# daveredrum/D3Net

Hardware: AMD Instinct MI355X
Metric: scenes/sec fwd+bwd (PointGroup+speaker) (higher is better)
Workload: dtype bf16

## Files before the change

### d3net_amd/_lib.py

```python
import ctypes as C
import os

_HERE = os.path.dirname(os.path.abspath(__file__))
SO_PATH = os.path.join(_HERE, "lib", "libd3hip.so")

ERRORS = {-1: "D3_ERR_WORKSPACE", -2: "D3_ERR_RANGE (coordinate/batch outside key range)",
          -3: "D3_ERR_ARG", -4: "D3_ERR_OVERFLOW"}


class D3Error(RuntimeError):
    pass


_lib = None
vp, i32, i64, f32, sz = C.c_void_p, C.c_int, C.c_longlong, C.c_float, C.c_size_t
f64 = C.c_double
pi = C.POINTER(C.c_int)

SIGNATURES = {
    "d3_version": (i32, []),
    "d3_arch": (C.c_char_p, []),
    "d3_sec_mean": (i32, [vp, vp, vp, i32, i32, vp]),
    "d3_sec_min": (i32, [vp, vp, vp, i32, i32, vp]),
    "d3_sec_max": (i32, [vp, vp, vp, i32, i32, vp]),
# ... 145 lines not shown
    "d3_multiview_fuse_ws_bytes": (sz, [i32, i32, i32]),
    "d3_multiview_fuse": (i32, [vp, i32, vp, vp, vp, i32, C.POINTER(f64), i32, i32, vp, i32, i32, vp, vp, vp, sz, vp]),
    "d3_enet_layers": (i32, [vp, i32]),
    "d3_enet_param_count": (i64, []),
    "d3_enet_preprocess": (i32, [vp, i32, i32, i32, vp, vp, i32, i32, vp, vp]),
    "d3_enet_ws_bytes": (sz, [i32, i32, i32]),
    "d3_enet_forward": (i32, [vp, i32, i32, i32, vp, i64, vp, i32, i32, vp, vp, sz, vp]),
    "d3_scan_limits": (i32, [pi, pi, pi, pi, pi]),
    "d3_scan_mesh_ws_bytes": (sz, [i32, i32]),
    "d3_scan_mesh": (i32, [vp, i32, vp, i32, C.POINTER(f64), vp, vp, vp, vp, sz, vp]),
    "d3_scan_labels_ws_bytes": (sz, [i32, i32, i32, i32, i32]),
    "d3_scan_labels": (i32, [vp, vp, i32, i32, vp, vp, i32, vp, vp, i32, i32, vp, vp, vp, vp, vp, vp, vp, vp, vp, sz, vp]),
    "d3_cider_ws_bytes": (sz, [i32, i32, i32]),
    "d3_cider_scores": (i32, [vp, i32, vp, vp, vp, vp, vp, i32, i32, vp, i32, vp, i32, i32, f64, i32, vp, vp, vp, sz, vp]),
    "d3_graph_edges": (i32, [vp, vp, i32, i32, i32, vp, vp, vp, vp, vp, vp, vp, vp, vp, vp, vp]),
    "d3_edgeconv_ws_bytes": (sz, [i32, i32, i32]),
    "d3_edgeconv_bwd_ws_bytes": (sz, [i32, i32, i32]),
    "d3_edgeconv_fwd": (i32, [vp, vp, vp, vp, vp, vp, vp, vp, vp, i32, i32, i32, i32, i32, vp, vp, vp, sz, vp]),
    "d3_edgeconv_bwd": (i32, [vp, vp, vp, vp, vp, vp, vp, vp, i32, i32, i32, i32, i32, vp, vp, vp, vp, vp, vp, vp, vp, vp, sz, vp]),
    "d3_query_locals_dist": (i32, [vp, vp, vp, i32, i32, i32, f32, i32, vp]),
    "d3_prof_enable": (i32, [i32]),
    "d3_net_set_chunks": (i32, [vp, vp, i32]),
    "d3_net_chunk_wait": (i32, [vp, i32, vp]),
    "d3_layernorm_fwd": (i32, [vp, vp, vp, vp, vp, vp, vp, i32, i32, f32, vp]),
    "d3_layernorm_ws_bytes": (sz, [i32, i32]),
    "d3_layernorm_bwd": (i32, [vp, vp, vp, vp, vp, vp, vp, vp, vp, i32, i32, vp, sz, vp]),
    "d3_tuning_set": (i32, [C.c_char_p, i32]),
    "d3_tuning_get": (i32, [C.c_char_p, vp]),
    "d3_tuning_count": (i32, []),
    "d3_tuning_name": (C.c_char_p, [i32]),
    "d3_prof_collect": (i32, [i32, C.POINTER(C.c_longlong), C.POINTER(C.c_double), C.POINTER(C.c_double),
                              C.POINTER(C.c_double)]),
    "d3_prof_dump": (i32, [i32, C.POINTER(C.c_double), i32, C.POINTER(i32)]),
    "d3_bn_ws_bytes": (sz, [i32]),
    "d3_bn_stats": (i32, [vp, i32, i32, vp, vp, vp, vp, f32, vp, sz, vp]),
    "d3_bn_relu_fwd": (i32, [vp, vp, vp, vp, vp, vp, i32, i32, f32, i32, vp]),
    "d3_bn_relu_fwd_bf16": (i32, [vp, vp, vp, vp, vp, vp, i32, i32, f32, i32, vp]),
    "d3_bn_relu_bwd": (i32, [vp, vp, vp, vp, vp, vp, vp, vp, vp, i32, i32, f32, i32, vp, sz, vp]),
}


class GemmSeg(C.Structure):
    _fields_ = [("A", vp), ("ia", vp), ("lda", i64), ("a_kmajor", i32), ("B", vp), ("ldb", i64), ("b_kmajor", i32), ("K", i32)]


class GemmProb(C.Structure):
# ... 63 lines not shown
```

### d3net_amd/csrc/unet.hip

```cpp
#include "conv.h"
#include <vector>
#include <map>
#include <string.h>
#include <stdlib.h>

__device__ __forceinline__ unsigned int un_pack2bf(float lo, float hi) {
    unsigned int a = __float_as_uint(lo), b = __float_as_uint(hi);
    a += 0x7FFFu + ((a >> 16) & 1u); b += 0x7FFFu + ((b >> 16) & 1u);
    return (a >> 16) | (b & 0xFFFF0000u);
}

__device__ __forceinline__ float un_ld1(const float *p, long long idx, int bf) {
    return bf ? __uint_as_float((unsigned int)((const unsigned short *)p)[idx] << 16) : p[idx];
}
__device__ __forceinline__ float4 un_ldx4(const float *x, long long idx, int xbf) {
    if (xbf) { const uint2 v = *(const uint2 *)((const unsigned short *)x + idx); return make_float4(__uint_as_float(v.x), __uint_as_float(v.y), 0.f, 0.f); }
    return *(const float4 *)(x + idx);
}
__device__ __forceinline__ void un_cvx4(const float4 r, int xbf, float *o) {
    if (xbf) {
        const unsigned int a = __float_as_uint(r.x), b = __float_as_uint(r.y);
        o[0] = __uint_as_float(a << 16); o[1] = __uint_as_float(a & 0xFFFF0000u); o[2] = __uint_as_float(b << 16); o[3] = __uint_as_float(b & 0xFFFF0000u);
    } else { o[0] = r.x; o[1] = r.y; o[2] = r.z; o[3] = r.w; }
}
// ... 543 lines not shown
}

enum { OP_CONV = 1, OP_BNACT = 2, OP_PADCAST = 3, OP_STATS = 4 };
enum { MAP_K1 = 0, MAP_K3 = 1, MAP_DOWN = 2, MAP_UP = 3 };

struct TensorD { int level, C, ld, coff, dtype, buf; };
struct BufD { int level, width, dtype; size_t off, goff; int need_grad; };
struct SrcRef { int op, c0, cn; };
struct OpD {
    int type, in, out, res, w, gamma, beta, rmean, rvar, map, mlevel, K, CinW, stats, relu;
    float eps, momentum;
    int Cin, Cout;
    size_t wp_fwd, wp_bwd, part_off, state_off;
    int nparts, partw;
    std::vector<SrcRef> srcs;
    int in_grad_mode;
    int res_mode;
    int needs_dgrad_pack;
    int bn_of_in;
    int fused_by;
    size_t bpart_off; int bparts;
    size_t part2_off, bpart2_off;
    int wg_hazard;
    size_t wpart_off, wpart_bytes; int wsplits;
    int use_shadow;
    int write_shadow;
};
#define RED_RING 32
struct Net {
    std::vector<TensorD> T;
    std::vector<BufD> B;
    std::vector<OpD> ops;
    int nlevels = 0, nparams = 0, input_needs_grad = 0, out_tensor = -1;
    std::vector<int> rows;
    std::vector<int> galias;
    std::vector<int> gbf;
    std::vector<int> gabf;
    std::vector<int> gshadow;
    std::vector<size_t> gshadow_off;
    size_t arena_bytes = 0, grad_bytes = 0, ws_bytes = 0, bnscr_off = 0, wgws_off = 0, bnscr_bytes = 0, wgws_bytes = 0;
    bool planned = false;
    bool f32 = false;
    size_t cnt_off0 = 0, cnt_bytes = 0, bcnt_off0 = 0, bcnt_bytes = 0;
    std::vector<PackJob> jobs;
    PackJob *jobs_dev = nullptr;
    size_t jobs_cap = 0;
    long long pack_total = 0;
    hipStream_t side = nullptr;
    hipStream_t side2 = nullptr;
    std::vector<hipEvent_t> ev;
    size_t ev_used = 0;
    int xp_op = -1;
    int xp_tensor = -1;
    const void *xp_ext = nullptr;
    std::vector<const void *> k3_16;
    std::vector<const void *> k3_q;
    std::vector<int> chunk_op;
    std::vector<hipEvent_t> chunk_ev_side, chunk_ev_main;
    RedJob *red_host = nullptr, *red_dev = nullptr;
    size_t red_cap = 0; int red_flip = 0;
    hipEvent_t next_event() {
        if (ev_used == ev.size()) { hipEvent_t e; if (hipEventCreateWithFlags(&e, hipEventDisableTiming) != hipSuccess) return nullptr; ev.push_back(e); }
        return ev[ev_used++];
    }
};

static int esize(int dtype) { return dtype == 1 ? 2 : 4; }

extern "C" void *d3_net_create(const int64_t *prog, int nops, const int64_t *tensors, int ntensors, const int64_t *bufs,
                               int nbufs, int nlevels, int nparams, int input_needs_grad, int out_tensor) {
    Net *n = new Net();
    n->nlevels = nlevels; n->nparams = nparams; n->input_needs_grad = input_needs_grad; n->out_tensor = out_tensor;
    for (int i = 0; i < ntensors; i++) {
        const int64_t *t = tensors + (size_t)i * 6;
        n->T.push_back(TensorD{(int)t[0], (int)t[1], (int)t[2], (int)t[3], (int)t[4], (int)t[5]});
    }
    for (int i = 0; i < nbufs; i++) {
        const int64_t *b = bufs + (size_t)i * 3;
        n->B.push_back(BufD{(int)b[0], (int)b[1], (int)b[2], 0, 0, 1});
    }
    n->f32 = true;
    for (auto &b : n->B) if (b.dtype == 1) n->f32 = false;
    for (int i = 0; i < nops; i++) {
        const int64_t *p = prog + (size_t)i * 16;
        OpD o;
        o.type = (int)p[0]; o.in = (int)p[1]; o.out = (int)p[2]; o.res = (int)p[3];
        o.w = o.gamma = o.beta = o.rmean = o.rvar = -1; o.map = 0; o.mlevel = 0; o.K = 1; o.CinW = 0; o.stats = 0; o.relu = 0;
        o.eps = 0.f; o.momentum = 0.f; o.Cin = o.Cout = 0; o.wp_fwd = o.wp_bwd = o.part_off = o.state_off = 0;
        o.nparts = 0; o.partw = 0; o.in_grad_mode = 0; o.res_mode = 0; o.needs_dgrad_pack = 0;
        o.bn_of_in = -1; o.fused_by = -1; o.bpart_off = 0; o.bparts = 0; o.part2_off = 0; o.bpart2_off = 0; o.wg_hazard = 0; o.wpart_off = 0; o.wpart_bytes = 0; o.wsplits = 1; o.use_shadow = 0; o.write_shadow = 0;
        if (o.type == OP_CONV) {
            o.w = (int)p[4]; o.map = (int)p[5]; o.mlevel = (int)p[6]; o.K = (int)p[7]; o.CinW = (int)p[8]; o.stats = (int)p[9];
            o.Cin = n->T[o.in].C; o.Cout = n->T[o.out].C;
        } else if (o.type == OP_BNACT) {
            o.gamma = (int)p[4]; o.beta = (int)p[5]; o.rmean = (int)p[6]; o.rvar = (int)p[7]; o.relu = (int)p[8];
            int32_t eb = (int32_t)p[9], mb = (int32_t)p[10];
            memcpy(&o.eps, &eb, 4); memcpy(&o.momentum, &mb, 4);
        } else if (o.type == OP_STATS) {
            o.stats = 1;
        }
        if (o.type == OP_PADCAST && n->xp_op < 0 && n->T[(size_t)o.in].buf < 0) { n->xp_op = (int)n->ops.size(); n->xp_tensor = o.out; }
        n->ops.push_back(o);
    }
    for (auto &o : n->ops) {
        if (o.type != OP_BNACT) continue;
        const TensorD &ti = n->T[o.in];
        for (size_t j = 0; j < n->ops.size(); j++) {
            const OpD &p = n->ops[j];
            if (!p.stats) continue;
            const TensorD &tp = n->T[p.type == OP_STATS ? p.in : p.out];
            if (tp.buf != ti.buf) continue;
            if (tp.coff >= ti.coff && tp.coff + tp.C <= ti.coff + ti.C) o.srcs.push_back(SrcRef{(int)j, tp.coff - ti.coff, tp.C});
        }
// ... 132 lines not shown
        };
        struct LastBn { int op, coff, C; };
        std::map<int, LastBn> last_bn;
        for (int i = (int)n->ops.size() - 1; on && i >= 0; i--) {
            OpD &o = n->ops[i];
            int coff, C;
            if (o.type == OP_CONV) {
                const int ro = root_of(o.out, coff, C);
                if (ro >= 0 && !n->gbf[ro] && !(C & 7)) {
                    auto it = last_bn.find(ro);
                    if (it != last_bn.end() && it->second.op >= 0 && it->second.coff == coff && it->second.C == C &&
                        (!n->gshadow[ro] || n->gshadow[ro] == C)) {
                        o.use_shadow = 1; n->ops[it->second.op].write_shadow = 1; n->gshadow[ro] = C;
                    }
                }
                if (o.in_grad_mode) { const int ri = root_of(o.in, coff, C); if (ri >= 0) last_bn[ri] = LastBn{-1, 0, 0}; }
                if (o.res >= 0 && o.res_mode >= 2) { const int rr = root_of(o.res, coff, C); if (rr >= 0) last_bn[rr] = LastBn{-1, 0, 0}; }
            } else if (o.type == OP_BNACT && o.in_grad_mode) {
                const int ri = root_of(o.in, coff, C);
                if (ri >= 0) last_bn[ri] = n->gbf[ri] ? LastBn{-1, 0, 0} : LastBn{i, coff, C};
            }
        }
    }
    {
        hipStreamCreateWithFlags(&n->side, hipStreamNonBlocking);
        hipStreamCreateWithFlags(&n->side2, hipStreamNonBlocking);
    }
    return n;
}

extern "C" void d3_net_destroy(void *h) {
    Net *n = (Net *)h;
    if (!n) return;
    if (n->jobs_dev) hipFree(n->jobs_dev);
    if (n->red_host) hipHostFree(n->red_host);
    if (n->red_dev) hipFree(n->red_dev);
    for (auto e : n->ev) hipEventDestroy(e);
    for (auto e : n->chunk_ev_side) hipEventDestroy(e);
    for (auto e : n->chunk_ev_main) hipEventDestroy(e);
    if (n->side) hipStreamDestroy(n->side);
    if (n->side2) hipStreamDestroy(n->side2);
    delete n;
}

extern "C" int d3_net_set_chunks(void *h, const int *op_idx, int nchunks) {
    Net *n = (Net *)h;
// ... 32 lines not shown
    Net *n = (Net *)h;
    const int Cd = d3_net_padded_channels(h);
    if (!n || Cd <= 0 || !input || !out || M < 0) return D3_ERR_ARG;
    const int Cs = n->T[(size_t)n->ops[(size_t)n->xp_op].in].C;
    const long long total = M * (Cd / 2);
    if (total > 0) un_padcast_kernel<<<(int)((total + 255) / 256), 256, 0, d3_stream(stream)>>>((const float *)input, (unsigned short *)out, M, Cs, Cd);
    D3_LAUNCH_CHECK();
    return 0;
}
extern "C" int d3_net_set_padded_input(void *h, const void *xp) {
    Net *n = (Net *)h;
    if (!n) return D3_ERR_ARG;
    n->xp_ext = d3_net_padded_channels(h) > 0 ? xp : nullptr;
    return 0;
}
extern "C" int d3_net_chunk_wait(void *h, int k, void *stream) {
    Net *n = (Net *)h;
    if (!n || k < 0 || k >= (int)n->chunk_op.size()) return D3_ERR_ARG;
    D3_CHECK(hipStreamWaitEvent(d3_stream(stream), n->chunk_ev_side[k], 0));
    D3_CHECK(hipStreamWaitEvent(d3_stream(stream), n->chunk_ev_main[k], 0));
    return 0;
}

static int bn_blocks2(int M, int C) {
    const int rpp = UN_T / C;
    long long blocks = ((long long)M + rpp - 1) / rpp;
    blocks = (blocks + 15) / 16;
    if (blocks < 1) blocks = 1;
    if (blocks > 512) blocks = 512;
    return (int)blocks;
}

static void conv_dims(const Net *n, const OpD &o, int &Min, int &Mout) {
    Min = n->rows[n->T[o.in].level]; Mout = n->rows[n->T[o.out].level];
}

extern "C" int d3_net_plan(void *h, const int *rows, size_t *arena_bytes, size_t *grad_bytes) {
    Net *n = (Net *)h;
    n->rows.assign(rows, rows + n->nlevels);
    size_t off = 0, goff = 0;
    for (auto &b : n->B) {
        b.off = off; off += d3_align((size_t)n->rows[b.level] * b.width * esize(b.dtype));
        const size_t bi = &b - &n->B[0];
        b.goff = goff; if (b.need_grad) goff += d3_align((size_t)n->rows[b.level] * b.width * ((n->gbf[bi] || n->gabf[bi]) ? 2 : 4));
        if (n->gshadow[bi]) { n->gshadow_off[bi] = goff; goff += d3_align((size_t)n->rows[b.level] * n->gshadow[bi] * 2); }
    }
    size_t bnscr = 0, wgws = 16;
    for (auto &o : n->ops) {
        if (o.type == OP_CONV) {
            int Min, Mout; conv_dims(n, o, Min, Mout);
            const int pf = n->f32 ? D3_CONV_F32 : 0;
            o.wp_fwd = off; off += d3_align(d3_spconv_pack_bytes_ex(o.K, o.Cin, o.Cout, pf));
            o.wp_bwd = off; if (o.needs_dgrad_pack) off += d3_align(d3_spconv_pack_bytes_ex(o.K, o.Cout, o.Cin, pf));
            if (o.stats) {
                o.nparts = d3_spconv_fwd2_nparts_ex(Mout, o.K, o.Cin, o.Cout, pf);
                o.partw = (o.Cout + 15) / 16 * 16;
                o.part_off = off; off += d3_align((size_t)o.nparts * 2 * o.partw * 4);
            }
// ... 18 lines not shown
        const OpD &cv = n->ops[o.fused_by];
        int Min, Mout; conv_dims(n, cv, Min, Mout);
        o.bparts = d3_spconv_fwd2_nparts_ex(Min, cv.K, cv.Cout, cv.CinW, n->f32 ? D3_CONV_F32 : 0);
        o.bpart_off = goff; goff += d3_align((size_t)o.bparts * 2 * ((cv.CinW + 15) / 16 * 16) * 4);
    }
    for (auto &o : n->ops) if (o.type == OP_CONV) { o.wpart_off = goff; goff += o.wpart_bytes; }
    n->cnt_off0 = off;
    off = d3_align(off);
    for (auto &o : n->ops)
        if ((o.type == OP_CONV || o.type == OP_STATS) && o.nparts > 0) { o.part2_off = off; off += d3_align((size_t)D3_P2_ROWS * 2 * o.partw * 8); }
    n->cnt_bytes = off - n->cnt_off0;
    n->bcnt_off0 = goff;
    goff = d3_align(goff);
    for (auto &o : n->ops) {
        if (o.type != OP_BNACT || o.fused_by < 0) continue;
        const OpD &cv = n->ops[o.fused_by];
        o.bpart2_off = goff; goff += d3_align((size_t)D3_P2_ROWS * 2 * ((cv.CinW + 15) / 16 * 16) * 8);
    }
    n->bcnt_bytes = goff - n->bcnt_off0;
    n->arena_bytes = off;
    n->bnscr_off = goff; goff += d3_align(bnscr); n->bnscr_bytes = bnscr;
    n->wgws_off = goff; goff += d3_align(wgws); n->wgws_bytes = wgws;
    n->grad_bytes = goff;
    n->planned = true;
    *arena_bytes = n->arena_bytes; *grad_bytes = n->grad_bytes;
    return 0;
}

extern "C" long long d3_net_tensor_offset(void *h, int tensor) {
    Net *n = (Net *)h;
    const TensorD &t = n->T[tensor];
    if (t.buf < 0) return -1;
    return (long long)(n->B[t.buf].off + (size_t)t.coff * esize(t.dtype));
}

struct Maps { const int *const *k3; const int *const *child; const int *const *up; };

static void conv_tables(const OpD &o, const Maps &m, const int *&tf, const int *&tb, int &bwd_flip) {
    tf = tb = nullptr; bwd_flip = 0;
    if (o.map == MAP_K3) { tf = tb = m.k3[o.mlevel]; bwd_flip = 1; }
    else if (o.map == MAP_DOWN) { tf = m.child[o.mlevel]; tb = m.up[o.mlevel]; }
    else if (o.map == MAP_UP) { tf = m.up[o.mlevel]; tb = m.child[o.mlevel]; }
}

static inline char *tptr(const Net *n, char *arena, const void *input, int tensor) {
    const TensorD &t = n->T[tensor];
// ... 174 lines not shown
}

static int net_backward_impl(void *h, const void *const *params, const int *const *k3, const int *const *child,
                             const int *const *up, const void *input, void *arena_, void *garena_, const float *gout,
                             float *const *pgrads, const int *paccum, float *gin, void *stream);
extern "C" int d3_net_backward(void *h, const void *const *params, const int *const *k3, const int *const *child,
                               const int *const *up, const void *input, void *arena_, void *garena_, const float *gout,
                               float *const *pgrads, const int *paccum, float *gin, void *stream) {
    if (!h) return D3_ERR_ARG;
    const int rc = net_backward_impl(h, params, k3, child, up, input, arena_, garena_, gout, pgrads, paccum, gin, stream);
    net_drop_k3_16((Net *)h);
    return rc;
}
static int net_backward_impl(void *h, const void *const *params, const int *const *k3, const int *const *child,
                             const int *const *up, const void *input, void *arena_, void *garena_, const float *gout,
                             float *const *pgrads, const int *paccum, float *gin, void *stream) {
    D3_CLEAR();
    Net *n = (Net *)h;
    if (!n->planned) return D3_ERR_ARG;
    hipStream_t s = d3_stream(stream);
    char *arena = (char *)arena_, *garena = (char *)garena_;
    Maps maps{k3, child, up};
    n->ev_used = 0;
    constexpr int kSideMinRows = 32768;
    const bool use_side = n->rows[0] >= kSideMinRows;
    hipStream_t ws_stream = use_side ? n->side : s;
    std::map<int, hipEvent_t> pending;
    bool side_used = false;
    bool main_wgrads = false;
    auto wait_pending = [&](int root) {
        if (!use_side) return;
        auto it = pending.find(root);
        if (it != pending.end()) { hipStreamWaitEvent(s, it->second, 0); pending.erase(it); }
    };
    if (n->bcnt_bytes) D3_CHECK(hipMemsetAsync(garena + n->bcnt_off0, 0, n->bcnt_bytes, s));
    const bool use_p2 = d3_tune(D3T_BN_PART2) != 0;
    float *bnscr = (float *)(garena + n->bnscr_off);
    std::vector<RedJob> red;
    long long red_blocks = 0;
    const bool use_side2 = use_side && n->side2;
    bool side2_dirty = false;
    int side2_flip = 0;
    auto join_side2 = [&]() -> int {
        if (!side2_dirty) return 0;
        hipEvent_t e = n->next_event();
        if (!e) return D3_ERR_OVERFLOW;
        D3_CHECK(hipEventRecord(e, n->side2));
// ... 8 lines not shown
            hipEvent_t e = n->next_event();
            if (!e) return D3_ERR_OVERFLOW;
            D3_CHECK(hipEventRecord(e, s));
            D3_CHECK(hipStreamWaitEvent(ws_stream, e, 0));
            main_wgrads = false;
        }
        if (red.size() > n->red_cap) {
            D3_CHECK(hipStreamSynchronize(ws_stream));
            if (n->red_host) hipHostFree(n->red_host);
            if (n->red_dev) hipFree(n->red_dev);
            n->red_cap = red.size() + 16;
            D3_CHECK(hipHostMalloc((void **)&n->red_host, RED_RING * n->red_cap * sizeof(RedJob)));
            D3_CHECK(hipMalloc((void **)&n->red_dev, RED_RING * n->red_cap * sizeof(RedJob)));
        }
        n->red_flip = (n->red_flip + 1) % RED_RING;
        RedJob *hj = n->red_host + (size_t)n->red_flip * n->red_cap, *dj = n->red_dev + (size_t)n->red_flip * n->red_cap;
        memcpy(hj, red.data(), red.size() * sizeof(RedJob));
        D3_CHECK(hipMemcpyAsync(dj, hj, red.size() * sizeof(RedJob), hipMemcpyHostToDevice, ws_stream));
        un_wgrad_reduce_batched_kernel<<<(int)red_blocks, 256, 0, ws_stream>>>(dj, (int)red.size());
        red.clear();
        red_blocks = 0;
        return 0;
    };
    constexpr int kRedTail = 5;
    int tail_idx = -1;
    for (int i = 0, c = 0; i < (int)n->ops.size(); i++)
        if (n->ops[i].type == OP_CONV && pgrads[n->ops[i].w] != nullptr && ++c == kRedTail) { tail_idx = i; break; }
    size_t next_chunk = 0;
    auto chunk_done = [&](int i) -> int {
        while (next_chunk < n->chunk_op.size() && n->chunk_op[next_chunk] >= i) {
            int frc = flush_red(); if (frc) return frc;
            frc = join_side2(); if (frc) return frc;
            D3_CHECK(hipEventRecord(n->chunk_ev_side[next_chunk], ws_stream));
            D3_CHECK(hipEventRecord(n->chunk_ev_main[next_chunk], s));
            next_chunk++;
        }
        return 0;
    };
    for (int i = (int)n->ops.size() - 1; i >= 0; i--) {
        OpD &o = n->ops[i];
        if (i < (int)n->ops.size() - 1) { int crc = chunk_done(i + 1); if (crc) return crc; }
        if (i == tail_idx) { int frc = flush_red(); if (frc) return frc; }
        if (o.type == OP_CONV) {
            const TensorD &ti = n->T[o.in];
            int Min, Mout; conv_dims(n, o, Min, Mout);
            const int *tf, *tb; int flip; conv_tables(o, maps, tf, tb, flip);
            int ldgo, root_o, gobf; float *go = gptr(n, garena, gout, gin, o.out, ldgo, root_o, &gobf);
            float *go32 = go;
            const int ldgo32 = ldgo;
            if (o.use_shadow && root_o >= 0 && n->gshadow[root_o]) { go = (float *)(garena + n->gshadow_off[root_o]); gobf = 1; ldgo = n->gshadow[root_o]; }
            const bool op_side = use_side;
            hipEvent_t e1 = nullptr;
            if (pgrads[o.w] != nullptr && op_side) {
                e1 = n->next_event();
                if (!e1) return D3_ERR_OVERFLOW;
                D3_CHECK(hipEventRecord(e1, s));
            }
            if (o.in_grad_mode) {
                int ldgi, root_i, gibf; float *gi = gptr(n, garena, gout, gin, o.in, ldgi, root_i, &gibf);
                const int obf = gibf ? D3_CONV_OUTBF16 : 0;
                if (root_i >= 0) wait_pending(root_i);
                ConvExtras ex;
                if (o.map == MAP_K3 && (size_t)o.mlevel < n->k3_16.size()) {
                    ex.tbl16 = n->k3_16[(size_t)o.mlevel];
                    if (use_p2 || o.bn_of_in < 0) ex.tblq = n->k3_q[(size_t)o.mlevel];
                }
                int rc, np = 0;
                if (o.bn_of_in >= 0) {
                    const OpD &b = n->ops[o.bn_of_in];
                    const TensorD &tx = n->T[b.in];
                    float *mean = (float *)(arena + b.state_off), *var = mean + tx.C;
                    if (use_p2) ex.part2 = (double *)(garena + b.bpart2_off);
                    const ConvBn bn{tptr(n, arena, input, b.in), mean, var, (const float *)params[b.gamma], (const float *)params[b.beta], tx.ld, b.relu, tx.dtype == 1 ? 1 : 0, b.eps};
                    rc = d3_conv2_run(go, ldgo, tb, arena + o.wp_bwd, gi, ldgi, nullptr, 0, (float *)(garena + b.bpart_off), Mout, Min, o.K, o.Cout, o.CinW,
                                      (gobf ? D3_CONV_XBF16 : 0) | (n->f32 ? D3_CONV_F32 : 0) | obf, &bn, ex, &np, stream);
                    if (!rc) n->ops[o.bn_of_in].bparts = np;
                } else {
                    rc = d3_conv2_run(go, ldgo, tb, arena + o.wp_bwd, gi, ldgi, nullptr, 0, nullptr, Mout, Min, o.K, o.Cout, o.CinW,
                                      (o.in_grad_mode == 2 ? D3_CONV_ACCUM : 0) | (gobf ? D3_CONV_XBF16 : 0) | (n->f32 ? D3_CONV_F32 : 0) | obf, nullptr, ex, &np, stream);
                }
                if (rc) return rc;
            }
            if (o.res_mode >= 2) {
                int ldr, root_r; float *gr = gptr(n, garena, gout, gin, o.res, ldr, root_r);
                if (root_r >= 0) wait_pending(root_r);
                const long long total = (long long)Mout * (o.Cout / 4);
                if (total > 0) un_add_kernel<<<(int)((total + 255) / 256), 256, 0, s>>>(gr, ldr, go32, ldgo32, Mout, o.Cout, o.res_mode == 3 ? 1 : 0);
            }
            if (pgrads[o.w] != nullptr) {
                if (!op_side) main_wgrads = true;
                hipStream_t wst = ws_stream;
                if (op_side) {
                    if (use_side2 && (side2_flip++ & 1)) { wst = n->side2; side2_dirty = true; }
                    D3_CHECK(hipStreamWaitEvent(wst, e1, 0));
                    side_used = true;
                }
                const bool xstat = o.Cin > o.Cout;
                int flags = (ti.dtype == 1 ? D3_CONV_XBF16 : 0) | (paccum[o.w] ? D3_CONV_ACCUM : 0) | (gobf ? D3_CONV_DYBF16 : 0) | (n->f32 ? D3_CONV_F32 : 0);
                const int *tw = tf;
                if (xstat) { flags |= D3_CONV_XSTAT | (flip ? D3_CONV_FLIPK : 0); tw = tb; }
                float *dW = pgrads[o.w];
                char *wpart = garena + o.wpart_off;
                const void *tw16 = (o.map == MAP_K3 && (size_t)o.mlevel < n->k3_16.size()) ? n->k3_16[(size_t)o.mlevel] : nullptr;
                int rc = d3_conv2_wgrad(tptr(n, arena, input, o.in), ti.ld, tw, tw16, go, ldgo, dW, Min, Mout, o.K, o.Cin, o.Cout, o.CinW,
                                        flags | D3_CONV_NOREDUCE, wpart, o.wpart_bytes, (void *)(op_side ? wst : s));
                if (o.wsplits > 1 || paccum[o.w] || n->f32) {
                    RedJob j;
                    memset(&j, 0, sizeof(j));
                    j.part = (const float *)wpart; j.dW = dW; j.n = (long long)o.K * o.CinW * o.Cout; j.R = o.wsplits;
                    j.accum = paccum[o.w] ? 1 : 0; j.start = red_blocks;
                    red_blocks += (j.n + 127) / 128;
                    red.push_back(j);
                }
                if (rc) return rc;
                if (op_side && root_o >= 0 && o.wg_hazard) {
                    auto prev = pending.find(root_o);
                    if (prev != pending.end()) D3_CHECK(hipStreamWaitEvent(wst, prev->second, 0));
                    hipEvent_t e2 = n->next_event();
                    if (!e2) return D3_ERR_OVERFLOW;
                    D3_CHECK(hipEventRecord(e2, wst));
                    pending[root_o] = e2;
                }
            }
        } else if (o.type == OP_BNACT) {
            if (!o.in_grad_mode && pgrads[o.gamma] == nullptr) continue;
            const TensorD &ti = n->T[o.in];
            const int M = n->rows[ti.level], C = ti.C;
            if (M <= 0) continue;
            float *mean = (float *)(arena + o.state_off), *var = mean + C, *sums = var + C;
            const float *gamma = (const float *)params[o.gamma], *beta = (const float *)params[o.beta];
            int ldgo, root_o, gobf; float *go = gptr(n, garena, gout, gin, o.out, ldgo, root_o, &gobf);
            const float *x = (const float *)tptr(n, arena, input, o.in);
            int relu = o.relu;
            const int fs_rows_b = d3_tune(D3T_BN_FUSED_ROWS);
            if (o.fused_by >= 0 && fs_rows_b > 0 && C <= UN_FS_MAXC &&
                (use_p2 || 2ll * o.bparts * C <= UN_FS_MAX_PART_FLOATS)) {
// ... 22 lines not shown
                un_bn_bwd_final_kernel<<<(C + 3) / 4, 256, 0, s>>>((const float *)(garena + o.bpart_off), o.bparts, C, sums,
                                                               pgrads[o.gamma], pgrads[o.beta], paccum[o.gamma]);
                relu = 0;
            } else {
                const int nb = bn_blocks2(M, C);
                un_bn_bwd_reduce_kernel<<<nb, UN_T, 0, s>>>(x, ti.ld, go, ldgo, mean, var, gamma, beta, M, C, o.eps, o.relu, bnscr, gobf, ti.dtype == 1 ? 1 : 0);
                un_bn_bwd_final_kernel<<<(C + 3) / 4, 256, 0, s>>>(bnscr, nb, C, sums, pgrads[o.gamma], pgrads[o.beta], paccum[o.gamma]);
            }
            if (o.in_grad_mode) {
                int ldgi, root_i, gibf; float *gi = gptr(n, garena, gout, gin, o.in, ldgi, root_i, &gibf);
                if (root_i >= 0) wait_pending(root_i);
                const long long total = (long long)M * (C / 4);
                unsigned short *sh = (o.write_shadow && root_i >= 0 && n->gshadow[root_i] == C) ? (unsigned short *)(garena + n->gshadow_off[root_i]) : nullptr;
#define UN_APB(OBFV, GBFV, ACC_, SH_)                                                                                                     \
                un_bn_bwd_apply_kernel<OBFV, GBFV><<<un_ap_grid(M, C, UN_AP_U * 2), 256, 0, s>>>(x, ti.ld, go, ldgo, mean, var, gamma, beta, sums, gi, ldgi, M, C, \
                                                                                              o.eps, relu, ACC_, SH_, ti.dtype == 1 ? 1 : 0)
                if (gibf) { if (gobf) UN_APB(true, true, 0, nullptr); else UN_APB(true, false, 0, nullptr); }
                else if (gobf) UN_APB(false, true, o.in_grad_mode == 2 ? 1 : 0, sh);
                else UN_APB(false, false, o.in_grad_mode == 2 ? 1 : 0, sh);
#undef UN_APB
            }
        }
    }
    { int frc = flush_red(); if (frc) return frc; }
    { int crc = chunk_done(0); if (crc) return crc; }
    { int jrc = join_side2(); if (jrc) return jrc; }
    if (side_used) {
        hipEvent_t e = n->next_event();
        if (!e) return D3_ERR_OVERFLOW;
        D3_CHECK(hipEventRecord(e, n->side));
        D3_CHECK(hipStreamWaitEvent(s, e, 0));
    }
    D3_LAUNCH_CHECK();
    return 0;
}
```

### d3net_amd/netexec.py

```python
import ctypes as C
import struct

import torch
from torch.autograd import Function

from . import _lib, common
from . import minkowski as ME
from ._lib import check
from .pointgroup_ops import _on, _stream

OP_CONV, OP_BNACT, OP_PADCAST, OP_STATS = 1, 2, 3, 4
MAP_K1, MAP_K3, MAP_DOWN, MAP_UP = 0, 1, 2, 3
F32, BF16 = 0, 1
import os as _os
SINGLE_READER_BF16 = _os.environ.get("D3X_T_F32", "") == ""


def _fbits(x):
    return struct.unpack("<i", struct.pack("<f", float(x)))[0]


class _Builder:
    def __init__(self, act_dtype=BF16):
        self.tensors, self.bufs, self.ops, self.params, self.grad_params, self.bns = [], [], [], [], [], []
        self.act_dtype = act_dtype

    def buf(self, level, width, dtype):
        self.bufs.append((level, width, dtype))
        return len(self.bufs) - 1

    def view(self, buf, coff, Cc):
        level, width, dtype = self.bufs[buf]
        self.tensors.append((level, Cc, width, coff, dtype, buf))
        return len(self.tensors) - 1

    def new(self, level, Cc, dtype):
        return self.view(self.buf(level, Cc, dtype), 0, Cc)

# ... 87 lines not shown
            x = b.conv(xp, stem, 0, cin_w=in_channels)
        else:
            b.op(OP_STATS, x)
        x = b.ublock(ublock, x)
        out = b.bnact(x, final_bn, out_dtype=F32, relu=final_bn.fused_relu)
        self.b = b
        self.out_tensor, self.out_channels = out, b.C(out)
        self.nlevels = len(ublock.nPlanes)
        self.input_needs_grad = bool(input_needs_grad)
        self.in_channels = in_channels
        self.handle = None
        self._ptr_key = None
        self._plan_key, self._plan = None, None
        self._flat_grad, self._grad_views = None, None
        self.fresh_grads = False
        self.debug_keep = False
        self.debug_last = None
        self.debug_pairs = None
        self.on_backward = None
        self.backward_done = False
        self.backward_count = 0
        self.forward_count = 0
        self._chunk_ranges = None

    def _net(self):
        if self.handle is None:
            b = self.b
            L = _lib.lib()
            prog = (C.c_int64 * (16 * len(b.ops)))(*[v for op in b.ops for v in op])
            tens = (C.c_int64 * (6 * len(b.tensors)))(*[v for t in b.tensors for v in t])
            bufs = (C.c_int64 * (3 * len(b.bufs)))(*[v for t in b.bufs for v in t])
            self.handle = C.c_void_p(L.d3_net_create(prog, len(b.ops), tens, len(b.tensors), bufs, len(b.bufs), self.nlevels,
                                                     len(b.params), int(self.input_needs_grad), self.out_tensor))
            assert self.handle.value
        return self.handle

    def __deepcopy__(self, memo):
        return None

    def __del__(self):
        try:
            if self.handle is not None and self.handle.value:
                _lib.lib().d3_net_destroy(self.handle)
        except Exception:
            pass

# ... 190 lines not shown
                if fresh:
                    if ps[i].grad is not v:
                        ps[i].grad = v
                else:
                    g = ps[i].grad
                    if g is None or g.data_ptr() != v.data_ptr():
                        ps[i].grad = v
                    else:
                        acc[i] = 1
        net.fresh_grads = False
        net._plan_for(ctx.rows)
        garena = torch.empty(ctx.grad_bytes, dtype=torch.uint8, device=dev)
        gin = torch.empty_like(ctx.feats) if net.input_needs_grad else None
        k16 = keep[-1]
        if ctx.cm is not None and not net.exact:
            n_ = net.nlevels
            ptrs = [(t.data_ptr() if t is not None else 0) for t in (ctx.cm.k3_16(1 << l) for l in range(n_))]
            qptrs = [(t.data_ptr() if t is not None else 0) for t in (ctx.cm.k3_q(1 << l) for l in range(n_))]
            k16 = ((C.c_void_p * n_)(*ptrs), (C.c_void_p * n_)(*qptrs))
        with _on(dev):
            check(L.d3_net_set_k3_16(net._net(), k16[0], k16[1]), "net_set_k3_16")
            if ctx.xp is not None:
                check(L.d3_net_set_padded_input(net._net(), C.c_void_p(ctx.xp.data_ptr())), "net_set_padded_input")
            check(L.d3_net_backward(net._net(), net._param_ptrs(), k3, child, up, C.c_void_p(ctx.feats.data_ptr()),
                                    C.c_void_p(ctx.arena.data_ptr()), C.c_void_p(garena.data_ptr()), C.c_void_p(gout.data_ptr()),
                                    pg, acc, C.c_void_p(gin.data_ptr()) if gin is not None else None, _stream()), "net_backward")
        net.backward_count += 1
        net.backward_done = True
        if net.on_backward is not None:
            net.on_backward(net)
        return (gin, None, None, None) + (None,) * (len(ctx.needs_input_grad) - 4)
```

### include/d3hip.h

```cpp
#ifndef D3HIP_H
#define D3HIP_H
#include <stddef.h>
#include <stdint.h>

#ifdef __cplusplus
extern "C" {
#endif

#define D3_ERR_WORKSPACE (-1)
#define D3_ERR_RANGE     (-2)
#define D3_ERR_ARG       (-3)
#define D3_ERR_OVERFLOW  (-4)

int d3_version(void);
const char *d3_arch(void);

int d3_sec_mean(const float *inp, const int *offsets, float *out, int nProposal, int C, void *stream);
int d3_sec_min(const float *inp, const int *offsets, float *out, int nProposal, int C, void *stream);
int d3_sec_max(const float *inp, const int *offsets, float *out, int nProposal, int C, void *stream);
int d3_cluster_select(const float *locs, const float *pt_offsets, const int64_t *semantic_preds, const int *batch_idxs,
                      const int64_t *object_idxs, int n, int *batch_out, float *coords_out, float *shifted_out, int *semantic_out,
                      void *stream);
int d3_cluster_select2(const float *locs, const float *pt_offsets, const int64_t *semantic_preds, const int *batch_idxs,
                       const int64_t *object_idxs, int n, int batch_size, int *batch_out, float *coords_out, float *shifted_out,
// ... 150 lines not shown
int d3_bn_relu_fwd_bf16(const float *x, const float *mean, const float *var, const float *gamma, const float *beta,
                        void *y_bf16, int M, int C, float eps, int relu, void *stream);
int d3_bn_relu_bwd(const float *x, const float *dy, const float *mean, const float *var, const float *gamma,
                   const float *beta, float *dx, float *dgamma, float *dbeta, int M, int C, float eps, int relu,
                   void *ws, size_t ws_bytes, void *stream);

void *d3_net_create(const int64_t *prog, int nops, const int64_t *tensors, int ntensors, const int64_t *bufs, int nbufs,
                    int nlevels, int nparams, int input_needs_grad, int out_tensor);
void d3_net_destroy(void *net);
int d3_net_plan(void *net, const int *rows, size_t *arena_bytes, size_t *grad_bytes);
long long d3_net_tensor_offset(void *net, int tensor);
int d3_net_forward(void *net, const void *const *params, const int *const *k3, const int *const *child,
                   const int *const *up, const void *input, void *arena, int training, void *stream);
int d3_net_backward(void *net, const void *const *params, const int *const *k3, const int *const *child,
                    const int *const *up, const void *input, void *arena, void *grad_arena, const float *gout,
                    float *const *pgrads, const int *paccum, float *gin, void *stream);
int d3_net_set_chunks(void *net, const int *op_idx, int nchunks);
int d3_net_set_k3_16(void *net, const void *const *k3_16, const int *const *k3_q);
int d3_net_padded_channels(void *net);
int d3_net_padcast(void *net, const void *input, void *out, long long M, void *stream);
int d3_net_set_padded_input(void *net, const void *xp);
long long d3_spconv_t16_launches(void);
int d3_net_chunk_wait(void *net, int k, void *stream);

size_t d3_tall_wgrad_ws_bytes(int I, int O);
int d3_tall_wgrad(const float *x, const float *dy, float *dW, float *db, int N, int I, int O, void *ws, size_t ws_bytes,
                  void *stream);
size_t d3_offset_loss_ws_bytes(void);
int d3_offset_loss(const float *pt, const float *coords, const float *info, int ldi, const int64_t *ids, long long ignore,
                   float *g1, float *g2, float *out, int N, void *ws, size_t ws_bytes, void *stream);
size_t d3_point_heads_ws_bytes(void);
int d3_point_heads_fwd(const float *x, long long N, int m, int C, const float *Ws, const float *bs, const float *W0, const float *b0,
                       const float *gamma, const float *beta, const float *W3, const float *b3, float eps, float momentum,
                       int training, float *running_mean, float *running_var, long long *num_batches_tracked, float *scores,
                       long long *preds, float *h, float *y, float *offsets, float *stat, void *ws, size_t ws_bytes, void *stream);
int d3_point_heads_dy(const float *g_off, const float *W3, const float *y, long long N, float *dy, void *stream);
int d3_point_heads_dx(const float *dh, const float *W0, const float *g_scores, const float *Ws, long long N, int C, float *dx,
                      void *stream);
int d3_score_loss(const float *scores, const float *ious, int P, int nInst, float fg, float bg, float *gt_iou,
                  float *dscore, float *out, void *stream);
size_t d3_masked_xe_ws_bytes(int N, int S);
int d3_masked_xe(const float *pred, const long long *target, long long ld_target, const unsigned char *good, int N, int S, int V,
                 float *dpred, float *out2, void *ws, size_t ws_bytes, void *stream);
int d3_orientation_loss(const float *preds, long long ld_batch, long long ld_edge, const float *edge_index,
                        const long long *num_src, const long long *num_tar, const long long *assign, const float *rotations,
                        const float *rot_masks, int B, int E, int K, int G, int num_bins, const float *bounds_host,
// ... 203 lines not shown
```

Measured before the change: 251.5.

## Defer small-conv weight-gradient launches and batch them onto side streams

In the sparse UNet backward pass, weight-gradient kernels for small convolutions (both row counts below a threshold) are no longer launched right after each op's dgrad. They are queued and flushed together at chunk boundaries, before large convs, or at the tail. Each flush uses one event and splits the kernels across the side streams. This cuts per-op event record/wait overhead and keeps small wgrad kernels off the main dgrad critical path. A plan-time hazard analysis (dy root not overwritten later, disjoint gradient buffers) limits which ops can be deferred, and a wrong analysis could produce stale gradients.

```diff
diff --git a/d3net_amd/_lib.py b/d3net_amd/_lib.py
--- a/d3net_amd/_lib.py
+++ b/d3net_amd/_lib.py
@@ -191,6 +191,8 @@
     "d3_prof_enable": (i32, [i32]),
     "d3_net_set_chunks": (i32, [vp, vp, i32]),
     "d3_net_chunk_wait": (i32, [vp, i32, vp]),
+    "d3_net_set_defer_wgrad": (i32, [vp, i32]),
+    "d3_net_deferred_wgrads": (i32, [vp]),
     "d3_layernorm_fwd": (i32, [vp, vp, vp, vp, vp, vp, vp, i32, i32, f32, vp]),
     "d3_layernorm_ws_bytes": (sz, [i32, i32]),
     "d3_layernorm_bwd": (i32, [vp, vp, vp, vp, vp, vp, vp, vp, vp, i32, i32, vp, sz, vp]),
diff --git a/d3net_amd/csrc/unet.hip b/d3net_amd/csrc/unet.hip
--- a/d3net_amd/csrc/unet.hip
+++ b/d3net_amd/csrc/unet.hip
@@ -589,11 +589,15 @@
     size_t bpart_off; int bparts;
     size_t part2_off, bpart2_off;
     int wg_hazard;
+    int dy_root;
+    int wg_late_ok;
+    int wg_defer;
     size_t wpart_off, wpart_bytes; int wsplits;
     int use_shadow;
     int write_shadow;
 };
 #define RED_RING 32
+struct DeferredWg { int op; float *go; int ldgo, gobf; };
 struct Net {
     std::vector<TensorD> T;
     std::vector<BufD> B;
@@ -626,6 +630,9 @@
     std::vector<hipEvent_t> chunk_ev_side, chunk_ev_main;
     RedJob *red_host = nullptr, *red_dev = nullptr;
     size_t red_cap = 0; int red_flip = 0;
+    std::vector<DeferredWg> deferred;
+    bool defer_wgrad = true, gbufs_disjoint = false;
+    int deferred_last = 0;
     hipEvent_t next_event() {
         if (ev_used == ev.size()) { hipEvent_t e; if (hipEventCreateWithFlags(&e, hipEventDisableTiming) != hipSuccess) return nullptr; ev.push_back(e); }
         return ev[ev_used++];
@@ -655,7 +662,7 @@
         o.w = o.gamma = o.beta = o.rmean = o.rvar = -1; o.map = 0; o.mlevel = 0; o.K = 1; o.CinW = 0; o.stats = 0; o.relu = 0;
         o.eps = 0.f; o.momentum = 0.f; o.Cin = o.Cout = 0; o.wp_fwd = o.wp_bwd = o.part_off = o.state_off = 0;
         o.nparts = 0; o.partw = 0; o.in_grad_mode = 0; o.res_mode = 0; o.needs_dgrad_pack = 0;
-        o.bn_of_in = -1; o.fused_by = -1; o.bpart_off = 0; o.bparts = 0; o.part2_off = 0; o.bpart2_off = 0; o.wg_hazard = 0; o.wpart_off = 0; o.wpart_bytes = 0; o.wsplits = 1; o.use_shadow = 0; o.write_shadow = 0;
+        o.bn_of_in = -1; o.fused_by = -1; o.bpart_off = 0; o.bparts = 0; o.part2_off = 0; o.bpart2_off = 0; o.wg_hazard = 0; o.dy_root = -1; o.wg_late_ok = 0; o.wg_defer = 0; o.wpart_off = 0; o.wpart_bytes = 0; o.wsplits = 1; o.use_shadow = 0; o.write_shadow = 0;
         if (o.type == OP_CONV) {
             o.w = (int)p[4]; o.map = (int)p[5]; o.mlevel = (int)p[6]; o.K = (int)p[7]; o.CinW = (int)p[8]; o.stats = (int)p[9];
             o.Cin = n->T[o.in].C; o.Cout = n->T[o.out].C;
@@ -834,6 +841,18 @@
             }
         }
     }
+    for (int i = 0; i < (int)n->ops.size(); i++) {
+        OpD &o = n->ops[i];
+        if (o.type != OP_CONV) continue;
+        const int r = o.dy_root = groot(o.out);
+        if (r < 0 || o.wg_hazard) continue;
+        o.wg_late_ok = 1;
+        for (int j = i - 1; j >= 0 && o.wg_late_ok; j--) {
+            const OpD &q = n->ops[j];
+            if ((q.type == OP_CONV || q.type == OP_BNACT) && q.in_grad_mode && groot(q.in) == r) o.wg_late_ok = 0;
+            if (q.type == OP_CONV && q.res >= 0 && q.res_mode >= 2 && groot(q.res) == r) o.wg_late_ok = 0;
+        }
+    }
     {
         hipStreamCreateWithFlags(&n->side, hipStreamNonBlocking);
         hipStreamCreateWithFlags(&n->side2, hipStreamNonBlocking);
@@ -912,6 +931,17 @@
     return 0;
 }
 
+extern "C" int d3_net_set_defer_wgrad(void *h, int on) {
+    Net *n = (Net *)h;
+    if (!n) return D3_ERR_ARG;
+    n->defer_wgrad = on != 0;
+    return 0;
+}
+extern "C" int d3_net_deferred_wgrads(void *h) {
+    Net *n = (Net *)h;
+    return n ? n->deferred_last : 0;
+}
+
 static int bn_blocks2(int M, int C) {
     const int rpp = UN_T / C;
     long long blocks = ((long long)M + rpp - 1) / rpp;
@@ -924,6 +954,9 @@
 static void conv_dims(const Net *n, const OpD &o, int &Min, int &Mout) {
     Min = n->rows[n->T[o.in].level]; Mout = n->rows[n->T[o.out].level];
 }
+
+constexpr int kSideMinRows = 32768;
+constexpr int kDeferMaxRows = 32768;
 
 extern "C" int d3_net_plan(void *h, const int *rows, size_t *arena_bytes, size_t *grad_bytes) {
     Net *n = (Net *)h;
@@ -988,6 +1021,21 @@
     n->bnscr_off = goff; goff += d3_align(bnscr); n->bnscr_bytes = bnscr;
     n->wgws_off = goff; goff += d3_align(wgws); n->wgws_bytes = wgws;
     n->grad_bytes = goff;
+    n->gbufs_disjoint = true;
+    {
+        size_t end = 0;
+        auto claim = [&](size_t lo, size_t bytes) { if (bytes) { if (lo < end) n->gbufs_disjoint = false; end = lo + bytes; } };
+        for (size_t bi = 0; bi < n->B.size(); bi++) {
+            const BufD &b = n->B[bi];
+            if (b.need_grad) claim(b.goff, (size_t)n->rows[b.level] * b.width * ((n->gbf[bi] || n->gabf[bi]) ? 2 : 4));
+            if (n->gshadow[bi]) claim(n->gshadow_off[bi], (size_t)n->rows[b.level] * n->gshadow[bi] * 2);
+        }
+    }
+    for (auto &o : n->ops) {
+        if (o.type != OP_CONV) continue;
+        int Min, Mout; conv_dims(n, o, Min, Mout);
+        o.wg_defer = o.wg_late_ok && n->gbufs_disjoint && n->B[(size_t)o.dy_root].need_grad && Min < kDeferMaxRows && Mout < kDeferMaxRows;
+    }
     n->planned = true;
     *arena_bytes = n->arena_bytes; *grad_bytes = n->grad_bytes;
     return 0;
@@ -1208,7 +1256,6 @@
     char *arena = (char *)arena_, *garena = (char *)garena_;
     Maps maps{k3, child, up};
     n->ev_used = 0;
-    constexpr int kSideMinRows = 32768;
     const bool use_side = n->rows[0] >= kSideMinRows;
     hipStream_t ws_stream = use_side ? n->side : s;
     std::map<int, hipEvent_t> pending;
@@ -1263,6 +1310,52 @@
         red_blocks = 0;
         return 0;
     };
+    auto enqueue_wgrad = [&](int i, float *go, int ldgo, int gobf, hipStream_t wst) -> int {
+        const OpD &o = n->ops[i];
+        const TensorD &ti = n->T[o.in];
+        int Min, Mout; conv_dims(n, o, Min, Mout);
+        const int *tf, *tb; int flip; conv_tables(o, maps, tf, tb, flip);
+        const bool xstat = o.Cin > o.Cout;
+        int flags = (ti.dtype == 1 ? D3_CONV_XBF16 : 0) | (paccum[o.w] ? D3_CONV_ACCUM : 0) | (gobf ? D3_CONV_DYBF16 : 0) | (n->f32 ? D3_CONV_F32 : 0);
+        const int *tw = tf;
+        if (xstat) { flags |= D3_CONV_XSTAT | (flip ? D3_CONV_FLIPK : 0); tw = tb; }
+        float *dW = pgrads[o.w];
+        char *wpart = garena + o.wpart_off;
+        const void *tw16 = (o.map == MAP_K3 && (size_t)o.mlevel < n->k3_16.size()) ? n->k3_16[(size_t)o.mlevel] : nullptr;
+        int rc = d3_conv2_wgrad(tptr(n, arena, input, o.in), ti.ld, tw, tw16, go, ldgo, dW, Min, Mout, o.K, o.Cin, o.Cout, o.CinW,
+                                flags | D3_CONV_NOREDUCE, wpart, o.wpart_bytes, (void *)wst);
+        if (o.wsplits > 1 || paccum[o.w] || n->f32) {
+            RedJob j;
+            memset(&j, 0, sizeof(j));
+            j.part = (const float *)wpart; j.dW = dW; j.n = (long long)o.K * o.CinW * o.Cout; j.R = o.wsplits;
+            j.accum = paccum[o.w] ? 1 : 0; j.start = red_blocks;
+            red_blocks += (j.n + 127) / 128;
+            red.push_back(j);
+        }
+        return rc;
+    };
+    const bool defer_on = use_side && n->defer_wgrad;
+    n->deferred.clear();
+    n->deferred_last = 0;
+    auto flush_deferred = [&]() -> int {
+        if (n->deferred.empty()) return 0;
+        hipEvent_t e = n->next_event();
+        if (!e) return D3_ERR_OVERFLOW;
+        D3_CHECK(hipEventRecord(e, s));
+        bool waits[2] = {false, false};
+        for (const DeferredWg &d : n->deferred) {
+            int w = 0;
+            if (use_side2 && (side2_flip++ & 1)) { w = 1; side2_dirty = true; }
+            hipStream_t wst = w ? n->side2 : ws_stream;
+            if (!waits[w]) { D3_CHECK(hipStreamWaitEvent(wst, e, 0)); waits[w] = true; }
+            side_used = true;
+            const int rc = enqueue_wgrad(d.op, d.go, d.ldgo, d.gobf, wst);
+            if (rc) return rc;
+        }
+        n->deferred_last += (int)n->deferred.size();
+        n->deferred.clear();
+        return 0;
+    };
     constexpr int kRedTail = 5;
     int tail_idx = -1;
     for (int i = 0, c = 0; i < (int)n->ops.size(); i++)
@@ -1270,7 +1363,8 @@
     size_t next_chunk = 0;
     auto chunk_done = [&](int i) -> int {
         while (next_chunk < n->chunk_op.size() && n->chunk_op[next_chunk] >= i) {
-            int frc = flush_red(); if (frc) return frc;
+            int frc = flush_deferred(); if (frc) return frc;
+            frc = flush_red(); if (frc) return frc;
             frc = join_side2(); if (frc) return frc;
             D3_CHECK(hipEventRecord(n->chunk_ev_side[next_chunk], ws_stream));
             D3_CHECK(hipEventRecord(n->chunk_ev_main[next_chunk], s));
@@ -1281,10 +1375,11 @@
     for (int i = (int)n->ops.size() - 1; i >= 0; i--) {
         OpD &o = n->ops[i];
         if (i < (int)n->ops.size() - 1) { int crc = chunk_done(i + 1); if (crc) return crc; }
-        if (i == tail_idx) { int frc = flush_red(); if (frc) return frc; }
+        if (i == tail_idx) { int frc = flush_deferred(); if (!frc) frc = flush_red(); if (frc) return frc; }
         if (o.type == OP_CONV) {
-            const TensorD &ti = n->T[o.in];
             int Min, Mout; conv_dims(n, o, Min, Mout);
+            const bool defer = defer_on && o.wg_defer && pgrads[o.w] != nullptr;
+            if (pgrads[o.w] != nullptr && !(Min < kDeferMaxRows && Mout < kDeferMaxRows)) { int frc = flush_deferred(); if (frc) return frc; }
             const int *tf, *tb; int flip; conv_tables(o, maps, tf, tb, flip);
             int ldgo, root_o, gobf; float *go = gptr(n, garena, gout, gin, o.out, ldgo, root_o, &gobf);
             float *go32 = go;
@@ -1292,7 +1387,7 @@
             if (o.use_shadow && root_o >= 0 && n->gshadow[root_o]) { go = (float *)(garena + n->gshadow_off[root_o]); gobf = 1; ldgo = n->gshadow[root_o]; }
             const bool op_side = use_side;
             hipEvent_t e1 = nullptr;
-            if (pgrads[o.w] != nullptr && op_side) {
+            if (pgrads[o.w] != nullptr && op_side && !defer) {
                 e1 = n->next_event();
                 if (!e1) return D3_ERR_OVERFLOW;
                 D3_CHECK(hipEventRecord(e1, s));
@@ -1328,7 +1423,9 @@
                 const long long total = (long long)Mout * (o.Cout / 4);
                 if (total > 0) un_add_kernel<<<(int)((total + 255) / 256), 256, 0, s>>>(gr, ldr, go32, ldgo32, Mout, o.Cout, o.res_mode == 3 ? 1 : 0);
             }
-            if (pgrads[o.w] != nullptr) {
+            if (defer) {
+                n->deferred.push_back(DeferredWg{i, go, ldgo, gobf});
+            } else if (pgrads[o.w] != nullptr) {
                 if (!op_side) main_wgrads = true;
                 hipStream_t wst = ws_stream;
                 if (op_side) {
@@ -1336,23 +1433,7 @@
                     D3_CHECK(hipStreamWaitEvent(wst, e1, 0));
                     side_used = true;
                 }
-                const bool xstat = o.Cin > o.Cout;
-                int flags = (ti.dtype == 1 ? D3_CONV_XBF16 : 0) | (paccum[o.w] ? D3_CONV_ACCUM : 0) | (gobf ? D3_CONV_DYBF16 : 0) | (n->f32 ? D3_CONV_F32 : 0);
-                const int *tw = tf;
-                if (xstat) { flags |= D3_CONV_XSTAT | (flip ? D3_CONV_FLIPK : 0); tw = tb; }
-                float *dW = pgrads[o.w];
-                char *wpart = garena + o.wpart_off;
-                const void *tw16 = (o.map == MAP_K3 && (size_t)o.mlevel < n->k3_16.size()) ? n->k3_16[(size_t)o.mlevel] : nullptr;
-                int rc = d3_conv2_wgrad(tptr(n, arena, input, o.in), ti.ld, tw, tw16, go, ldgo, dW, Min, Mout, o.K, o.Cin, o.Cout, o.CinW,
-                                        flags | D3_CONV_NOREDUCE, wpart, o.wpart_bytes, (void *)(op_side ? wst : s));
-                if (o.wsplits > 1 || paccum[o.w] || n->f32) {
-                    RedJob j;
-                    memset(&j, 0, sizeof(j));
-                    j.part = (const float *)wpart; j.dW = dW; j.n = (long long)o.K * o.CinW * o.Cout; j.R = o.wsplits;
-                    j.accum = paccum[o.w] ? 1 : 0; j.start = red_blocks;
-                    red_blocks += (j.n + 127) / 128;
-                    red.push_back(j);
-                }
+                const int rc = enqueue_wgrad(i, go, ldgo, gobf, op_side ? wst : s);
                 if (rc) return rc;
                 if (op_side && root_o >= 0 && o.wg_hazard) {
                     auto prev = pending.find(root_o);
@@ -1421,7 +1502,7 @@
             }
         }
     }
-    { int frc = flush_red(); if (frc) return frc; }
+    { int frc = flush_deferred(); if (!frc) frc = flush_red(); if (frc) return frc; }
     { int crc = chunk_done(0); if (crc) return crc; }
     { int jrc = join_side2(); if (jrc) return jrc; }
     if (side_used) {
diff --git a/d3net_amd/netexec.py b/d3net_amd/netexec.py
--- a/d3net_amd/netexec.py
+++ b/d3net_amd/netexec.py
@@ -14,6 +14,7 @@
 F32, BF16 = 0, 1
 import os as _os
 SINGLE_READER_BF16 = _os.environ.get("D3X_T_F32", "") == ""
+DEFER_WGRAD = 1
 
 
 def _fbits(x):
@@ -147,6 +148,8 @@
         self.backward_count = 0
         self.forward_count = 0
         self._chunk_ranges = None
+        self.defer_wgrad = None
+        self.deferred_wgrads = 0
 
     def _net(self):
         if self.handle is None:
@@ -383,11 +386,13 @@
             check(L.d3_net_set_k3_16(net._net(), k16[0], k16[1]), "net_set_k3_16")
             if ctx.xp is not None:
                 check(L.d3_net_set_padded_input(net._net(), C.c_void_p(ctx.xp.data_ptr())), "net_set_padded_input")
+            check(L.d3_net_set_defer_wgrad(net._net(), int(bool(DEFER_WGRAD if net.defer_wgrad is None else net.defer_wgrad))), "net_set_defer_wgrad")
             check(L.d3_net_backward(net._net(), net._param_ptrs(), k3, child, up, C.c_void_p(ctx.feats.data_ptr()),
                                     C.c_void_p(ctx.arena.data_ptr()), C.c_void_p(garena.data_ptr()), C.c_void_p(gout.data_ptr()),
                                     pg, acc, C.c_void_p(gin.data_ptr()) if gin is not None else None, _stream()), "net_backward")
         net.backward_count += 1
         net.backward_done = True
+        net.deferred_wgrads = L.d3_net_deferred_wgrads(net._net())
         if net.on_backward is not None:
             net.on_backward(net)
         return (gin, None, None, None) + (None,) * (len(ctx.needs_input_grad) - 4)
diff --git a/include/d3hip.h b/include/d3hip.h
--- a/include/d3hip.h
+++ b/include/d3hip.h
@@ -196,6 +196,8 @@
 int d3_net_set_padded_input(void *net, const void *xp);
 long long d3_spconv_t16_launches(void);
 int d3_net_chunk_wait(void *net, int k, void *stream);
+int d3_net_set_defer_wgrad(void *net, int on);
+int d3_net_deferred_wgrads(void *net);
 
 size_t d3_tall_wgrad_ws_bytes(int I, int O);
 int d3_tall_wgrad(const float *x, const float *dy, float *dW, float *db, int N, int I, int O, void *ws, size_t ws_bytes,
```

Measured after the change: 248.0. -1.4%, worse.
